# prototypefund/your-voice-TTS

Hardware: AMD Instinct MI355X
Metric: mel-frames/sec + RTF, Tacotron2 + 60-iter Griffin-Lim, LJSpeech (higher is better)
Workload: dtype f32; 1 GPU; configs[1]: Tacotron2 single sentence, HIP decoder loop + HIP Griffin-Lim 60 iters; sentences_per_gpu=1, L=100, gl_iters=60, model_config=config_tacotron2.json + forward_attn_mask (synthesize.py:86), parallelism=single GPU

## Files before the change

your-voice-tts_amd/csrc/resident_decoder.hip:

```cpp
#include "handoff.h"
#include "resident.h"

namespace tts {
namespace {
using namespace handoff;

__device__ __forceinline__ float lstm_cell16(float pre, float& c) {
    const int k = threadIdx.x;
    const float act = (k >> 2) == 2 ? tanh_cell(pre) : sigmoid_cell(pre);
    const float f = dpp_move<0x104, 0xf>(act, 0.f);
    const float g = dpp_move<0x108, 0xf>(act, 0.f);
    const float o = dpp_move<0x10C, 0xf>(act, 0.f);
    const float c2 = f * c + act * g;
    c = c2;
    return o * tanh_cell(c2);
}
__device__ __forceinline__ float sigmoid_fast(float x) {
    return __builtin_amdgcn_rcpf(1.f + __builtin_amdgcn_exp2f(-x * 1.4426950408889634f));
}

__device__ __forceinline__ float dot4(float4 w, float4 x, float acc) {
    acc = fmaf(w.x, x.x, acc);
    acc = fmaf(w.y, x.y, acc);
    acc = fmaf(w.z, x.z, acc);
    return fmaf(w.w, x.w, acc);
}
__device__ __forceinline__ float4 ld4(const float* p) { return *reinterpret_cast<const float4*>(p); }
__device__ __forceinline__ void pin4(float4& a, float4& b, float4& c, float4& d) {
    asm volatile("" : "+v"(a.x), "+v"(a.y), "+v"(a.z), "+v"(a.w), "+v"(b.x), "+v"(b.y), "+v"(b.z), "+v"(b.w), "+v"(c.x),
                 "+v"(c.y), "+v"(c.z), "+v"(c.w), "+v"(d.x), "+v"(d.y), "+v"(d.z), "+v"(d.w));
}
__device__ __forceinline__ float sum32_dpp(float v) {
    v += dpp_move<0x111, 0xf>(v, 0.f);
    v += dpp_move<0x112, 0xf>(v, 0.f);
    v += dpp_move<0x114, 0xf>(v, 0.f);
    v += dpp_move<0x118, 0xf>(v, 0.f);
    v += dpp_move<0x142, 0xa>(v, 0.f);
    return v;
}

__device__ __forceinline__ int res_window(int k, int nn, int L) {
    if (k == 0) return nn >= 2 ? nn - 2 : nn - 2 + L;
    const int clo = nn >= 1 ? nn - 1 : L - 1, chi = min(nn + 2, L - 1);
    const int p = clo + k - 1;
    return p <= chi ? p : -1;
}
__device__ __forceinline__ int res_candidate(int s, int nn, int np, int L) {
    if (s < 5) return res_window(s, nn, L);
    if (s >= 15) return -1;
    const int p = res_window((s - 5) >> 1, np, L);
    if (p < 0) return -1;
    const int q = p + ((s - 5) & 1);
    return q < L ? q : -1;
}

__device__ __forceinline__ int res_part_slot(int sl, int k) { return sl * 32 + k; }

struct ResWin {
    int cx, clo, chi;
    bool in[4];
    bool iscx[4];
    bool pre, post;
};
__device__ __forceinline__ ResWin res_win(int n, int L) {
    ResWin w;
    w.cx = n >= 2 ? n - 2 : n - 2 + L;
    w.clo = n >= 1 ? n - 1 : L - 1;
    w.chi = min(n + 2, L - 1);
#pragma unroll
    for (int k = 0; k < 4; ++k) {
        w.in[k] = w.clo + k <= w.chi;
        w.iscx[k] = w.in[k] && w.clo + k == w.cx;
    }
    w.pre = w.cx < w.clo;
    w.post = w.cx > w.chi;
    return w;
}
__device__ __forceinline__ void res_weights(const ResWin& w, float rm, const float (&c)[4], float& wcx, float (&ww)[4]) {
    float aw[4];
#pragma unroll
    for (int k = 0; k < 4; ++k) aw[k] = (w.in[k] && !w.iscx[k]) ? c[k] : 0.f;
    const float rs = ((aw[0] + aw[1]) + aw[2]) + aw[3];
    const float vx = 0.01f * rm;
    const float denom = rs + vx;
    const float inv = 1.f / denom;
    wcx = vx * inv;
#pragma unroll
    for (int k = 0; k < 4; ++k) ww[k] = aw[k] * inv;
}
__device__ __forceinline__ float res_context(const ResWin& w, float wcx, const float (&ww)[4], float ex,
                                             const float (&erow)[4]) {
    const float px = wcx * ex;
    float ctx = 0.f;
    ctx = w.pre ? ctx + px : ctx;
#pragma unroll
    for (int k = 0; k < 4; ++k) {
        const float s = ctx + (w.iscx[k] ? px : ww[k] * erow[k]);
        ctx = w.in[k] ? s : ctx;
    }
    ctx = w.post ? ctx + px : ctx;
    return ctx;
}
template <bool SEL = false>
__device__ __forceinline__ float res_weight_at(const ResWin& w, float wcx, const float (&ww)[4], int p) {
    int d = p - w.clo;
    if (SEL) asm volatile("" : "+v"(d));
    const float w0 = ww[0], w1 = ww[1], w2 = ww[2], w3 = ww[3];
    float v = w0;
    v = d == 1 ? w1 : v;
    v = d == 2 ? w2 : v;
    v = d >= 3 ? w3 : v;
    v = (d >= 0 && p <= w.chi) ? v : 0.f;
    return p == w.cx ? wcx : v;
}
__device__ __forceinline__ int res_tail_next(const ResWin& w, float wcx, const float (&ww)[4], int L, float& tail) {
    tail = res_weight_at<true>(w, wcx, ww, L - 2) + res_weight_at<true>(w, wcx, ww, L - 1);
    float bv = 0.f;
    int bi = -1;
    auto consider = [&](bool present, int p, float wp) {
        const bool take = present && p <= L - 2 && wp > bv;
        bv = take ? wp : bv;
        bi = take ? p : bi;
    };
    consider(w.pre, w.cx, wcx);
#pragma unroll
    for (int k = 0; k < 4; ++k) consider(w.in[k], w.clo + k, w.iscx[k] ? wcx : ww[k]);
    consider(w.post, w.cx, wcx);
    return bi >= 0 ? bi + 1 : 0;
}

constexpr int SM_WDL = 16 * 16 * 32 * 4;
constexpr int SM_ST = 64;
constexpr int SM_RQ = 4 * 64 * 4;
constexpr int SM_RM = 2 * 6 * 64 * 4 + 2 * 256;
constexpr int SM_PROF = 2 * 16;
constexpr int SM_FLOATS = SM_WDL + HATT + HDEC + (ENC + 16) + PRE + ADIM + 16 + 16 + SM_ST + SM_RQ + SM_RM + SM_PROF + PRE;
static_assert(SM_RQ >= 3 * RES_LMAX + 2 * RES_WAVES + 16 + ADIM, "synthesis form: attention scratch");
static_assert(SM_RQ >= 2 * (RES_LMAX + 32) + RES_LMAX + RES_WAVES, "general attention form: weights, energies");
static_assert(SM_RM >= 2 * 6 * 64 * 4 + RES_LMAX + 32, "general attention form: cumulative weights");
static_assert(HDEC >= 4 * RES_LMAX, "full evaluation: four waves' partials in xh_dec");
static_assert(RES_LMAX == 4 * 64 && RES_LMAX == 32 * RES_WAVES, "4 positions per lane, one per wave of 32 CUs");

template <bool PROF, bool GEN>
__global__ __launch_bounds__(RES_THREADS, 1) void resident_decoder_kernel(const ResArgs a) {
    const int c = blockIdx.x;
    const int tid = threadIdx.x, lane = tid & 63;
    const int wave = __builtin_amdgcn_readfirstlane(tid >> 6);
    const int r = tid >> 5, ks = tid & 31;
    extern __shared__ __align__(16) float sm[];
    float4* wdl = reinterpret_cast<float4*>(sm);
    float* xh_att = sm + SM_WDL;
    float* xh_dec = xh_att + HATT;
    float* xctx = xh_dec + HDEC;
    float* xpre = xctx + ENC + 16;
    float* xq = xpre + PRE;
    float* gates = xq + ADIM;
    int* flags = reinterpret_cast<int*>(gates + 16);
    float* st = gates + 32;
    float* rq = st + SM_ST;
    float* rm = rq + SM_RQ;
    float* abuf = rq;
    float* an = abuf + 2 * RES_LMAX;
    float* scr = an + RES_LMAX;
    float* xv = scr + 2 * RES_WAVES + 16;
    long long* pacc = reinterpret_cast<long long*>(rm + SM_RM);
    float* xp1 = rm + SM_RM + SM_PROF;
    constexpr int GW_PAD = RES_LMAX + 32;
    float* gw = rq;
    float* geg = rq + 2 * GW_PAD;
    float* gts = geg + RES_LMAX;
    float* gcum = rm + 2 * 6 * 64 * 4;
    bool prof = false;
    long long plast = 0;
    long long* trace = PROF && a.prof ? a.prof + 2 * RES_PHASES + (size_t)c * RES_TRACE_STEPS * RES_TRACE_EV : nullptr;
#define RES_EV(t, k)                                                                                \
    if (PROF && trace && (t) < RES_TRACE_STEPS) trace[(t) * RES_TRACE_EV + (k)] = (long long)wall_clock64();
#define RES_MARK(k)                                     \
    if (PROF && prof && tid == 0) {                     \
        const long long now = (long long)wall_clock64(); \
        pacc[k] += now - plast;                         \
        plast = now;                                    \
    }

    float4 wa[14], wdc[4];
    constexpr int KF = HDEC + ENC;
    {
        const float4* p = a.w.wa + (size_t)c * 14 * RES_THREADS + tid;
#pragma unroll
        for (int i = 0; i < 14; ++i) wa[i] = p[(size_t)i * RES_THREADS];
        const float4* q = a.w.wdc + (size_t)c * 4 * RES_THREADS + tid;
#pragma unroll
        for (int i = 0; i < 4; ++i) wdc[i] = q[(size_t)i * RES_THREADS];
        if (wave == 2 && c < a.nmel)
            for (int i = 0; i < 6; ++i) reinterpret_cast<float4*>(rm)[i * 64 + lane] = ld4(a.w.wf + (size_t)c * KF + i * 256 + lane * 4);
        const float4* l = a.w.wdl + (size_t)c * (SM_WDL / 4);
        for (int i = tid; i < SM_WDL / 4; i += RES_THREADS) wdl[i] = l[i];
    }
    if (tid < 16) {
        st[tid] = a.w.ba[c * 16 + tid];
        st[16 + tid] = a.w.bd[c * 16 + tid];
    }
    if (tid < 4) {
        st[32 + tid] = a.c_att[4 * c + tid];
        st[36 + tid] = a.c_dec[4 * c + tid];
    }
    if (tid == 0) st[48] = c < a.nmel ? a.w.bf[c] : 0.f;
    if (tid == 1) st[49] = a.w.bf[a.nmel + PRE];
    for (int k = tid; k < HATT; k += RES_THREADS) {
        xh_att[k] = a.h_att[a.hps + k];
        xh_dec[k] = a.h_dec[a.hps + k];
    }
    for (int k = tid; k < ENC; k += RES_THREADS) xctx[k] = a.xa[PRE + k];
    if (tid == 0) {
        flags[0] = 0;
        flags[1] = 0;
        flags[5] = 0;
        for (int k = 0; k < RES_PHASES; ++k) pacc[k] = 0;
    }
    __syncthreads();
    const long long tmo = a.timeout_ticks;
    int xcc;
    asm volatile("s_getreg_b32 %0, hwreg(HW_REG_XCC_ID)" : "=s"(xcc));
    xcc &= 7;
    const unsigned setup_tag = (a.salt << 14) | 0x3FFFu;
    if (tid == 0) publish(a.gran + GR_SETUP + c, setup_tag, __int_as_float(xcc));
    if (wave == 0) {
        float v4[4];
        const bool ok = sweep<4, !GEN>(a.gran, setup_tag, v4, [&](int i) { return GR_SETUP + lane * 4 + i; }, tmo);
        int rank = 0, nx = 0, nmin = RES_CUS, nmax = 0;
        const int xref = __builtin_amdgcn_readfirstlane(__float_as_int(v4[0]) & 7);
        for (int k = 0; k < 8; ++k) {
            int cnt = 0;
#pragma unroll
            for (int i = 0; i < 4; ++i) {
                const int x = __float_as_int(v4[i]) & 7;
                cnt += __popcll(__ballot(x == k));
                if (k == xcc) rank += __popcll(__ballot(x == k && lane * 4 + i < c));
            }
            if (k == xcc) nx = cnt;
            if (cnt > 0) nmin = min(nmin, cnt);
            nmax = max(nmax, cnt);
        }
        if (GEN && nmax > RES_MIN_CUS_PER_XCD) nmin = 0;
        if (lane == 0) {
            int* fl = reinterpret_cast<int*>(flags);
            fl[2] = rank;
            fl[3] = nx;
            fl[4] = xref;
            if (!ok) { flags[1] = 1; fail(a.status, 6); }
            else if (nmin < RES_MIN_CUS_PER_XCD) { flags[1] = 1; fail(a.status, RES_STATUS_PLACEMENT); }
        }
    }
    __syncthreads();
    if (flags[1]) return;
    const int rank = flags[2], nx = flags[3];
    const int p2lo = rank * PRE / nx, p2hi = (rank + 1) * PRE / nx;
    const int r0 = p2lo + wave;
    const bool has_row = r0 < p2hi;
    const float4 wp0 = has_row ? ld4(a.w.w2 + r0 * PRE + lane * 4) : float4{0.f, 0.f, 0.f, 0.f};
    const float bp1 = has_row ? a.w.bf[a.nmel + r0] : 0.f;
    const float bp2 = has_row ? a.w.b2[r0] : 0.f;
    const float* w1p = a.w.wf + (size_t)(a.nmel + (has_row ? r0 : 0)) * KF + lane * 4;
    const bool stop_cu = rank == 0;
    if (stop_cu && wave == 3)
        for (int i = 0; i < 6; ++i)
            reinterpret_cast<float4*>(rm)[(6 + i) * 64 + lane] = ld4(a.w.wf + (size_t)(a.nmel + PRE) * KF + i * 256 + lane * 4);
    const int qrow = GEN ? 4 * rank + (wave >> 1) : rank + 32 * (wave >> 1), qhalf = wave & 1;
    const float4 wq0 = ld4(a.w.wq + qrow * HATT + qhalf * 512 + lane * 4);
    const float4 wq1 = ld4(a.w.wq + qrow * HATT + qhalf * 512 + 256 + lane * 4);
    const int L = a.L;
    const bool xlog = xcc == flags[4];
    const bool att_log = !GEN && xlog && rank == nx - 1;
    prof = PROF && a.prof != nullptr && a.prof_marks && (c == 0 || att_log);
    if (prof && tid == 0) plast = (long long)wall_clock64();
    int n = 0, n_prev = 0;
    float ufa = 0.f, vb = 0.f, ex = 0.f, erow[4] = {0.f, 0.f, 0.f, 0.f}, ptc = 0.f;
    const auto renc = __builtin_amdgcn_make_buffer_rsrc(const_cast<float*>(a.enc), (short)0, L * ENC * 4, 0x00020000);
    const auto rpt = __builtin_amdgcn_make_buffer_rsrc(const_cast<float*>(a.Pt), (short)0, ADIM * a.Lcap * 4, 0x00020000);
    auto prefetch_rows = [&](int nn) {
        const int cx = nn >= 2 ? nn - 2 : nn - 2 + L, clo = nn >= 1 ? nn - 1 : L - 1, chi = min(nn + 2, L - 1);
        ex = __uint_as_float(__builtin_amdgcn_raw_buffer_load_b32(renc, (cx * ENC + tid) * 4, 0, VOLATILE_AUX));
#pragma unroll
        for (int k = 0; k < 4; ++k)
            erow[k] = __uint_as_float(__builtin_amdgcn_raw_buffer_load_b32(
                renc, clo + k <= chi ? ((clo + k) * ENC + tid) * 4 : OOB_OFF, 0, VOLATILE_AUX));
    };
    auto advance_rows = [&](int from, int nn) {
        if (nn == from) return;
        if (nn == from + 1 && from >= 1) {
            ex = erow[0];
            erow[0] = erow[1];
            erow[1] = erow[2];
            erow[2] = erow[3];
            erow[3] = __uint_as_float(__builtin_amdgcn_raw_buffer_load_b32(
                renc, nn + 2 <= L - 1 ? ((nn + 2) * ENC + tid) * 4 : OOB_OFF, 0, VOLATILE_AUX));
        } else {
            prefetch_rows(nn);
        }
    };
    if constexpr (!GEN) {
        n = a.nidx[0];
        ufa = a.u[0];
        vb = a.v_b[0];
        for (int j = tid; j < L; j += RES_THREADS) abuf[j] = a.alpha[j];
        if (tid < ADIM) xv[tid] = a.v[tid];
        prefetch_rows(n);
    }
    const int gf = GEN ? a.gen : 0;
    const int s_e = GR_EX + xcc * RES_LMAX;
    float gu = 0.5f, gtb = 0.f;
    int gwin = -1, gn = 1;
    float gv0 = 0.f, gv1 = 0.f, gp0 = 0.f, gp1 = 0.f, gl0 = 0.f, gl1 = 0.f;
    float gtw[3];
#pragma unroll
    for (int k = 0; k < 3; ++k) gtw[k] = 0.f;
    auto gen_location = [&](const float* wrow) {
        const int pe = rank + 32 * wave;
        if (pe >= L) return;
        const float* src = (lane < 32 ? wrow : gcum) + pe + 1;
        const float4* wc = reinterpret_cast<const float4*>(a.loc_conv) + lane * 8;
        float sacc = 0.f;
#pragma unroll
        for (int q = 0; q < 8; q += 2) {
            const float4 w0 = wc[q], w1_ = wc[q + 1];
            sacc = fmaf(w0.x, src[4 * q], sacc);
            sacc = fmaf(w0.y, src[4 * q + 1], sacc);
            sacc = fmaf(w0.z, src[4 * q + 2], sacc);
            sacc = fmaf(w0.w, src[4 * q + 3], sacc);
            sacc = fmaf(w1_.x, src[4 * q + 4], sacc);
            sacc = fmaf(w1_.y, src[4 * q + 5], sacc);
            sacc = fmaf(w1_.z, src[4 * q + 6], sacc);
            sacc = fmaf(w1_.w, src[4 * q + 7], sacc);
            asm volatile("" ::: "memory");
        }
        const float tot = sacc + __shfl_xor(sacc, 32, 64);
        const float4* wd0 = reinterpret_cast<const float4*>(a.loc_dense + lane * NLOC);
        const float4* wd1 = reinterpret_cast<const float4*>(a.loc_dense + (lane + 64) * NLOC);
        float l0 = 0.f, l1 = 0.f;
#pragma unroll
        for (int q = 0; q < 8; ++q) {
            const float4 u0 = wd0[q], u1 = wd1[q];
            const float f0 = __int_as_float(__builtin_amdgcn_readlane(__float_as_int(tot), 4 * q));
            const float f1 = __int_as_float(__builtin_amdgcn_readlane(__float_as_int(tot), 4 * q + 1));
            const float f2 = __int_as_float(__builtin_amdgcn_readlane(__float_as_int(tot), 4 * q + 2));
            const float f3 = __int_as_float(__builtin_amdgcn_readlane(__float_as_int(tot), 4 * q + 3));
            l0 = fmaf(u0.x, f0, l0); l0 = fmaf(u0.y, f1, l0); l0 = fmaf(u0.z, f2, l0); l0 = fmaf(u0.w, f3, l0);
            l1 = fmaf(u1.x, f0, l1); l1 = fmaf(u1.y, f1, l1); l1 = fmaf(u1.z, f2, l1); l1 = fmaf(u1.w, f3, l1);
            asm volatile("" ::: "memory");
        }
        gl0 = l0;
        gl1 = l1;
    };
    if constexpr (GEN) {
        vb = a.v_b[0];
        gu = a.u[0];
        gn = a.nidx[0];
        if (gf & GEN_WINDOW) gwin = a.win0[0];
        if (gf & GEN_TA) {
            gtb = a.ta_b[0];
#pragma unroll
            for (int k = 0; k < 3; ++k) gtw[k] = a.ta_w[3 * tid + k];
        }
        gv0 = a.v[lane];
        gv1 = a.v[lane + 64];
        const int pe = rank + 32 * wave;
        if (pe < L) {
            gp0 = a.Pt[(int64_t)lane * a.Lcap + pe];
            gp1 = a.Pt[(int64_t)(lane + 64) * a.Lcap + pe];
        }
        for (int k = tid; k < GW_PAD; k += RES_THREADS) {
            const int j = k - 16;
            const bool ok = j >= 0 && j < L;
            gw[k] = ok ? a.alpha[j] : 0.f;
            gw[GW_PAD + k] = ok && (gf & GEN_LOCATION) ? a.att_w0[j] : 0.f;
            gcum[k] = ok && (gf & GEN_LOCATION) ? a.att_cum0[j] : 0.f;
        }
        __syncthreads();
        if (gf & GEN_LOCATION) gen_location(gw + GW_PAD);
    }
    const bool stop_lane = stop_cu && wave == 3 && lane == 0;
    if (stop_lane) {
        reinterpret_cast<int*>(st)[50] = a.flag1[0];
        reinterpret_cast<int*>(st)[51] = a.count[0];
    }
    u64* Gx = a.gran + GR_PRE2X + xcc * PRE;
    u64* Gq = a.gran + GR_QX + xcc * 2 * ADIM;
    u64* Gc = a.gran + GR_CTXX + xcc * GR_CTXX_STRIDE;
    u64* G1 = a.gran + GR_P1X + xcc * GR_P1X_STRIDE;
    const auto rg = __builtin_amdgcn_make_buffer_rsrc(a.gran, (short)0, 2 * GR_TOTAL * 8, 0x00020000);
    const int s_x = GR_PRE2X + xcc * PRE, s_q = GR_QX + xcc * 2 * ADIM, s_c = GR_CTXX + xcc * GR_CTXX_STRIDE,
              s_1 = GR_P1X + xcc * GR_P1X_STRIDE;
    const int pk = wave * 64 + lane;
    auto mel_row = [&](int tt) {
        if (c >= a.nmel) return;
        const float4* wm = reinterpret_cast<const float4*>(rm) + lane;
        float sm_ = 0.f;
#pragma unroll
        for (int i = 0; i < 4; ++i) sm_ = dot4(wm[i * 64], ld4(xh_dec + i * 256 + lane * 4), sm_);
#pragma unroll
        for (int i = 4; i < 6; ++i) sm_ = dot4(wm[i * 64], ld4(xctx + (i - 4) * 256 + lane * 4), sm_);
        sm_ = wave_sum_dpp(sm_);
        if (lane == 0 && tt < a.hist_cap) a.mel_hist[(int64_t)tt * a.nmel + c] = sm_ + st[48];
    };
#define RES_ATT_PARTIAL(out)                                                                                        \
    {                                                                                                               \
        float aa[2] = {0.f, 0.f};                                                                                   \
        _Pragma("unroll") for (int i = 2; i < 6; ++i)                                                               \
            aa[i & 1] = dot4(wa[i], ld4(xctx + (i - 2) * 128 + ks * 4), aa[i & 1]);                                 \
        _Pragma("unroll") for (int i = 6; i < 10; ++i)                                                              \
            aa[i & 1] = dot4(wa[i], ld4(xh_att + (i - 6) * 128 + ks * 4), aa[i & 1]);                               \
        asm volatile("" ::: "memory");                         \
        _Pragma("unroll") for (int i = 10; i < 14; ++i)                                                             \
            aa[i & 1] = dot4(wa[i], ld4(xh_att + (i - 6) * 128 + ks * 4), aa[i & 1]);                               \
        out = aa[0] + aa[1];                                                                                        \
    }
#define RES_DEC_PARTIAL(out)                                                                                        \
    {                                                                                                               \
        float ad[2] = {0.f, 0.f};                                                                                   \
        _Pragma("unroll 2") for (int i = 8; i < 16; ++i)                                                            \
            ad[i & 1] = dot4(wdl[(i * 16 + r) * 32 + ks], ld4(xh_dec + (i - 8) * 128 + ks * 4), ad[i & 1]);         \
        out = ad[0] + ad[1];                                                                                        \
    }
    float acc_a_next = 0.f;
    if constexpr (!GEN) RES_ATT_PARTIAL(acc_a_next)
    int t = 0;
    for (;; ++t) {
        u64* G = a.gran + (t & 1) * GR_TOTAL;
        u64* const gxs = GEN ? Gx + (t & 1) * GR_TOTAL : G + s_x;
        u64* const gqs = GEN ? Gq + (t & 1) * GR_TOTAL : G + s_q;
        u64* const gcs = GEN ? Gc + (t & 1) * GR_TOTAL : G + s_c;
        u64* const g1s = GEN ? G1 + (t & 1) * GR_TOTAL : G + s_1;
        const unsigned E = (a.salt << 14) | (((unsigned)t & 2047u) << 3);
        const unsigned EP6 = ((a.salt << 14) | (((unsigned)(t - 1) & 2047u) << 3)) + 6u;
        float acc_a, acc_d;
        if constexpr (GEN) {
            RES_ATT_PARTIAL(acc_a)
            RES_DEC_PARTIAL(acc_d)
        } else {
            acc_a = acc_a_next;
        }
        if (tid == 0) { RES_EV(t, 12) }
        if (tid == 192) { RES_EV(t, 13) }
        if (wave < 3) {
            const int gp = s_1 + ((t & 1) ^ 1) * GR_TOTAL;
            bool ok = true;
            if (t == 0) {
                if (wave == 0) {
                    const float4 v = ld4(a.pre1 + lane * 4);
                    xp1[lane * 4] = v.x; xp1[lane * 4 + 1] = v.y; xp1[lane * 4 + 2] = v.z; xp1[lane * 4 + 3] = v.w;
                }
            } else {
                float p0 = 0.f, p1 = 0.f;
                for (int i = 0; i < a.sleep_p1; ++i) __builtin_amdgcn_s_sleep(4);
                if (wave < 2) {
                    ok = sweep_pair(rg, gp + 2 * pk, true, EP6, p0, p1, tmo);
                    xp1[2 * pk] = p0;
                    xp1[2 * pk + 1] = p1;
                } else {
                    ok = sweep_pair(rg, lane == 0 ? gp + PRE : -1, false, EP6, p0, p1, tmo);
                    if (lane == 0 && ok && p0 == 0.f) flags[0] = 1;
                }
            }
            RES_MARK(0);
            if (lane == 0 && !ok) { flags[1] = 1; fail(a.status, 1, t); }
        }
        __syncthreads();
        if (tid == 0) { RES_EV(t, 0) }
        if (flags[0] | flags[1]) break;
        {
            const float4 x = ld4(xp1 + lane * 4);
            u64* gx = gxs;
            if (has_row) {
                const float s0 = wave_sum_dpp(dot4(wp0, x, 0.f));
                if (lane == 0) publish_xcd(gx + r0, E + 1, fmaxf(s0 + bp2, 0.f));
            }
            RES_MARK(1);
            if (wave < 2) {
                for (int i = 0; i < a.sleep_pre2; ++i) __builtin_amdgcn_s_sleep(4);
                float q0, q1;
                const bool ok = sweep_pair(rg, s_x + (t & 1) * GR_TOTAL + 2 * pk, true, E + 1, q0, q1, tmo);
                xpre[2 * pk] = q0;
                xpre[2 * pk + 1] = q1;
                if (!ok && lane == 0) { flags[1] = 1; fail(a.status, 7, t); }
            }
        }
        __syncthreads();
        if (tid == 0) { RES_EV(t, 1) }
        if (flags[1]) break;
        RES_MARK(2);
#pragma unroll
        for (int i = 0; i < 2; ++i) acc_a = dot4(wa[i], ld4(xpre + i * 128 + ks * 4), acc_a);
        acc_a = sum32_dpp(acc_a);
        if (ks == 31) gates[r] = acc_a;
        __syncthreads();
        RES_MARK(3);
        if (tid < 16) {
            float cs = st[32 + (tid & 3)];
            const float h = lstm_cell16(gates[tid] + st[tid], cs);
            if (tid < 4) {
                st[32 + tid] = cs;
                st[40 + tid] = h;
                publish(G + GR_HATT + 4 * c + tid, E + 2, h);
                if (tid == 0) { RES_EV(t, 2) }
            }
        }
        if (!GEN && t > 0) {
            advance_rows(n_prev, n);
            if (wave == 0) {
                const int pos = res_candidate(lane & 15, n, n_prev, L);
                ptc = __uint_as_float(__builtin_amdgcn_raw_buffer_load_b32(
                    rpt, pos >= 0 ? ((rank + 32 * (lane >> 4)) * a.Lcap + pos) * 4 : OOB_OFF, 0, VOLATILE_AUX));
            }
        }
        {
            if constexpr (!GEN) {
                RES_DEC_PARTIAL(acc_d)
                asm volatile("" : "+v"(acc_d));
            }
            if (wave == 4 && t > 0) mel_row(t - 1);
            for (int i = 0; i < a.sleep_hatt; ++i) __builtin_amdgcn_s_sleep(4);
            float h0, h1;
            const bool ok = sweep_pair(rg, (t & 1) * GR_TOTAL + GR_HATT + 2 * pk, true, E + 2, h0, h1, tmo);
            xh_att[2 * pk] = h0;
            xh_att[2 * pk + 1] = h1;
            if (!ok && lane == 0) { flags[1] = 1; fail(a.status, 2, t); }
        }
        __syncthreads();
        if (tid == 0) { RES_EV(t, 3) }
        if (flags[1]) break;
        RES_MARK(4);
        {
            float s = dot4(wq0, ld4(xh_att + qhalf * 512 + lane * 4), 0.f);
            s = dot4(wq1, ld4(xh_att + qhalf * 512 + 256 + lane * 4), s);
            s = wave_sum_dpp(s);
            if constexpr (GEN) {
                if (lane == 0) publish_xcd(gqs + 2 * qrow + qhalf, E + 3, s);
                if (tid == 0) { RES_EV(t, 8) }
            } else {
                if (lane == 0) scr[2 * wave] = s;
            }
        }
        if constexpr (!GEN) {
            __syncthreads();
            if (wave == 0 && t > 0) {
                const int m = lane >> 4;
                const float q = scr[4 * m] + scr[4 * m + 2];
                const float term = __fmul_rn(xv[rank + 32 * m], tanh_fast(__fadd_rn(q, ptc)));
                const float t1 = __shfl(term, (lane & 15) + 16, 64), t2 = __shfl(term, (lane & 15) + 32, 64),
                            t3 = __shfl(term, (lane & 15) + 48, 64);
                const float part = __fadd_rn(__fadd_rn(__fadd_rn(__fadd_rn(0.f, term), t1), t2), t3);
                if (lane < 16) publish_xcd(gcs + res_part_slot(lane, rank), E + 3, part);
                if (tid == 0) { RES_EV(t, 8) }
            }
        }
        if constexpr (!GEN) {
#pragma unroll 1
            for (int h = 0; h < 8; h += 4) {
                float4 wv[4], xx[4];
#pragma unroll
                for (int j = 0; j < 4; ++j) {
                    wv[j] = wdl[((h + j) * 16 + r) * 32 + ks];
                    xx[j] = ld4(xh_att + (h + j) * 128 + ks * 4);
                }
                pin4(wv[0], wv[1], wv[2], wv[3]);
                pin4(xx[0], xx[1], xx[2], xx[3]);
#pragma unroll
                for (int j = 0; j < 4; ++j) acc_d = dot4(wv[j], xx[j], acc_d);
            }
        } else {
#pragma unroll 2
            for (int i = 0; i < 8; ++i) acc_d = dot4(wdl[(i * 16 + r) * 32 + ks], ld4(xh_att + i * 128 + ks * 4), acc_d);
        }
        RES_MARK(5);
        float wcx = 0.f, ww[4] = {0.f, 0.f, 0.f, 0.f};
        if constexpr (GEN) {
            float2 gen_e[4];
#pragma unroll
            for (int i = 0; i < 4; ++i) {
                const int ps = (i >> 1) * 128 + 2 * lane + (i & 1);
                gen_e[i] = __builtin_bit_cast(float2, __builtin_amdgcn_raw_buffer_load_b64(
                    renc, ps < L ? (ps * ENC + 16 * rank + 2 * wave) * 4 : OOB_OFF, 0, VOLATILE_AUX));
            }
            if (wave < 2) {
                for (int i = 0; i < a.sleep_q; ++i) __builtin_amdgcn_s_sleep(1);
                float q0, q1;
                const bool ok = sweep_pair(rg, s_q + (t & 1) * GR_TOTAL + 2 * pk, true, E + 3, q0, q1, tmo);
                xq[pk] = q0 + q1;
                if (!ok && lane == 0) { flags[1] = 1; fail(a.status, 3, t); }
            }
            __syncthreads();
            if (flags[1]) break;
            if (rank + 32 * wave < L) {
                float x0 = xq[lane], x1 = xq[lane + 64];
                if (gf & GEN_LOCATION) {
                    x0 += gl0;
                    x1 += gl1;
                }
                const float e = wave_sum_dpp(gv0 * tanh_fast(x0 + gp0) + gv1 * tanh_fast(x1 + gp1));
                if (lane == 0) publish_xcd(a.gran + (t & 1) * GR_TOTAL + s_e + rank + 32 * wave, E + 7, e + vb);
            }
            if (wave < 2) {
                for (int i = 0; i < a.sleep_e; ++i) __builtin_amdgcn_s_sleep(1);
                const int p0 = 2 * pk;
                float e0 = 0.f, e1 = 0.f;
                const bool ok =
                    sweep_pair(rg, p0 < L ? s_e + (t & 1) * GR_TOTAL + p0 : -1, p0 + 1 < L, E + 7, e0, e1, tmo);
                geg[p0] = e0;
                geg[p0 + 1] = e1;
                if (!ok && lane == 0) { flags[1] = 1; fail(a.status, 8, t); }
            }
            __syncthreads();
            if (flags[1]) break;
            RES_MARK(6);
            const float* wold = gw + (t & 1) * GW_PAD + 16;
            float* wnew = gw + ((t & 1) ^ 1) * GW_PAD + 16;
            int ps[4];
            bool in[4];
            float e[4];
            {
                const float2 g0 = *reinterpret_cast<const float2*>(geg + 2 * lane);
                const float2 g1 = *reinterpret_cast<const float2*>(geg + 128 + 2 * lane);
                e[0] = g0.x; e[1] = g0.y; e[2] = g1.x; e[3] = g1.y;
            }
#pragma unroll
            for (int i = 0; i < 4; ++i) {
                ps[i] = (i >> 1) * 128 + 2 * lane + (i & 1);
                in[i] = ps[i] < L;
                if (!in[i]) e[i] = -INFINITY;
            }
            if (gf & GEN_WINDOW) {
                const int back = gwin - 2, front = gwin + 6;
#pragma unroll
                for (int i = 0; i < 4; ++i)
                    if (in[i] && ((back > 0 && ps[i] < back) || (front < L && ps[i] >= front))) e[i] = -INFINITY;
                if (gwin == -1) {
                    const float m = wave_max_dpp(fmaxf(fmaxf(e[0], e[1]), fmaxf(e[2], e[3])));
                    if (lane == 0) e[0] = m;
                }
                float bv = e[0];
                int bi = ps[0];
#pragma unroll
                for (int i = 1; i < 4; ++i)
                    if (e[i] > bv) { bv = e[i]; bi = ps[i]; }
                wave_argmax(bv, bi);
                gwin = __builtin_amdgcn_readfirstlane(bi);
            }
            float al[4];
            if (gf & GEN_SOFTMAX) {
                const float m = wave_max_dpp(fmaxf(fmaxf(e[0], e[1]), fmaxf(e[2], e[3])));
#pragma unroll
                for (int i = 0; i < 4; ++i) al[i] = in[i] ? expf(e[i] - m) : 0.f;
            } else {
#pragma unroll
                for (int i = 0; i < 4; ++i) al[i] = in[i] ? sigmoidf_(e[i]) : 0.f;
            }
            {
                const float S = wave_sum_dpp((al[0] + al[1]) + (al[2] + al[3]));
#pragma unroll
                for (int i = 0; i < 4; ++i) al[i] = al[i] / S;
            }
            if ((gf & GEN_LOCATION) && wave == 0) {
                float2* c01 = reinterpret_cast<float2*>(gcum + 16 + 2 * lane);
                float2* c23 = reinterpret_cast<float2*>(gcum + 16 + 128 + 2 * lane);
                const float2 o01 = *c01, o23 = *c23;
                *c01 = float2{o01.x + al[0], o01.y + al[1]};
                *c23 = float2{o23.x + al[2], o23.y + al[3]};
            }
            float w[4];
            if (gf & GEN_FORWARD) {
                float an[4];
#pragma unroll
                for (int i = 0; i < 4; ++i) {
                    const float ao = wold[ps[i]], pv = wold[ps[i] - 1];
                    const float mix = __fadd_rn(__fadd_rn(__fmul_rn(1.f - gu, ao), __fmul_rn(gu, pv)), 1e-8f);
                    an[i] = in[i] ? __fmul_rn(mix, al[i]) : 0.f;
                }
                if (gf & GEN_MASK) {
                    const float rmax = wave_max_dpp(fmaxf(fmaxf(in[0] ? an[0] : -INFINITY, in[1] ? an[1] : -INFINITY),
                                                          fmaxf(in[2] ? an[2] : -INFINITY, in[3] ? an[3] : -INFINITY)));
                    const int cx = gn >= 2 ? gn - 2 : gn - 2 + L, lo = gn >= 1 ? gn - 1 : L - 1;
#pragma unroll
                    for (int i = 0; i < 4; ++i) {
                        const bool keep = in[i] && ps[i] < gn + 3 && ps[i] >= lo;
                        an[i] = ps[i] == cx ? 0.01f * rmax : (keep ? an[i] : 0.f);
                    }
                }
                const float denom = wave_sum_dpp((an[0] + an[1]) + (an[2] + an[3]));
#pragma unroll
                for (int i = 0; i < 4; ++i) w[i] = in[i] ? an[i] / denom : 0.f;
                if (gf & GEN_MASK) {
                    float bv = -1.f;
                    int bi = 0x7fffffff;
#pragma unroll
                    for (int i = 0; i < 4; ++i)
                        if (ps[i] <= L - 2 && w[i] > bv) { bv = w[i]; bi = ps[i]; }
                    wave_argmax(bv, bi);
                    gn = __builtin_amdgcn_readfirstlane(bv > 0.f ? bi + 1 : 0);
                }
            } else {
#pragma unroll
                for (int i = 0; i < 4; ++i) w[i] = al[i];
            }
            RES_MARK(7);
            const float tail = wave_sum_dpp(((ps[0] >= L - 2 && in[0] ? w[0] : 0.f) + (ps[1] >= L - 2 && in[1] ? w[1] : 0.f)) +
                                            ((ps[2] >= L - 2 && in[2] ? w[2] : 0.f) + (ps[3] >= L - 2 && in[3] ? w[3] : 0.f)));
            float c0 = 0.f, c1 = 0.f;
#pragma unroll
            for (int i = 0; i < 4; ++i) {
                c0 = fmaf(w[i], gen_e[i].x, c0);
                c1 = fmaf(w[i], gen_e[i].y, c1);
            }
            c0 = wave_sum_dpp(c0);
            c1 = wave_sum_dpp(c1);
            {
                u64* gcx = gcs;
                if (lane < 2) publish_xcd(gcx + 16 * rank + 2 * wave + lane, E + 4, lane ? c1 : c0);
                if (rank == 0 && wave == 0 && lane == 2) publish_xcd(gcx + ENC, E + 4, tail);
            }
            if (tid == 0) { RES_EV(t, 11) }
            RES_MARK(8);
            if (wave == 0) {
                *reinterpret_cast<float2*>(wnew + 2 * lane) = float2{w[0], w[1]};
                *reinterpret_cast<float2*>(wnew + 128 + 2 * lane) = float2{w[2], w[3]};
                if (xlog && rank == 0 && t < a.hist_cap) {
#pragma unroll
                    for (int i = 0; i < 4; ++i)
                        if (ps[i] < a.Lalign) a.align_hist[(int64_t)t * a.Lalign + ps[i]] = w[i];
                }
            }
        }
        if constexpr (!GEN) {
            const float* aold = abuf + (t & 1) * RES_LMAX;
            float* candv = scr + 2 * RES_WAVES;
            const ResWin win = res_win(n, L);
            const int sl = tid >> 5, sub = tid & 31;
            const int pos = t > 0 ? res_candidate(sl, n, n_prev, L) : -1;
            const float a_pos = pos >= 0 ? aold[pos] : 0.f, a_prev = pos > 0 ? aold[pos - 1] : 0.f;
            const float mix = __fadd_rn(__fadd_rn(__fmul_rn(1.f - ufa, a_pos), __fmul_rn(ufa, a_prev)), 1e-8f);
            RES_MARK(9);
            bool full = t == 0;
            float rm = -INFINITY;
            float cw[4] = {0.f, 0.f, 0.f, 0.f};
            if (!full) {
                for (int i = 0; i < a.sleep_q; ++i) __builtin_amdgcn_s_sleep(1);
                float part = 0.f;
                const bool ok = sweep_one(rg, s_c + (t & 1) * GR_TOTAL + res_part_slot(sl, sub), E + 3, part, tmo);
                if (!ok && lane == 0) { flags[1] = 1; fail(a.status, 10, t); }
                if (tid == 0) { RES_EV(t, 9) }
                RES_MARK(6);
                const float e = sum32_dpp(part);
                if (sub == 31) {
                    const float v = pos >= 0 ? __fmul_rn(mix, sigmoid_fast(e + vb)) : -INFINITY;
                    if (pos >= 0) an[pos] = v;
                    candv[sl] = v;
                }
                __syncthreads();
                if (tid == 0) { RES_EV(t, 10) }
                if (flags[1]) break;
                RES_MARK(14);
                const float cand = candv[lane & 15];
                rm = wave_max_dpp(cand);
                full = !(rm >= 1e-8f);
#pragma unroll
                for (int k = 0; k < 4; ++k) cw[k] = __int_as_float(__builtin_amdgcn_readlane(__float_as_int(cand), 1 + k));
            }
            if (full) {
                const unsigned F = (a.salt << 14) | (((unsigned)flags[5] & 2047u) << 3) | 3u;
                if (lane == 0) publish_xcd(gqs + 2 * qrow + qhalf, F, scr[2 * wave]);
                if (wave < 2) {
                    float q0, q1;
                    const bool ok = sweep_pair(rg, s_q + (t & 1) * GR_TOTAL + 2 * pk, true, F, q0, q1, tmo);
                    xq[pk] = q0 + q1;
                    if (!ok && lane == 0) { flags[1] = 1; fail(a.status, 3, t); }
                }
                __syncthreads();
                if (flags[1]) break;
                if (tid == 0) flags[5] += 1;
                float xqd[16];
#pragma unroll
                for (int dd = 0; dd < 16; ++dd) xqd[dd] = xq[16 * wave + dd];
                float* red = xh_dec;
                const int j = tid;
                float e = 0.f;
#pragma unroll 1
                for (int h = 0; h < 2; ++h) {
                    if ((wave >> 2) == h) {
#pragma unroll 1
                        for (int jj = lane; jj < L; jj += 64) {
                            float s = 0.f;
#pragma unroll
                            for (int dd = 0; dd < 16; ++dd) {
                                const int d = 16 * wave + dd;
                                s += xv[d] * tanh_fast(xqd[dd] + a.Pt[(int64_t)d * a.Lcap + jj]);
                            }
                            red[(wave & 3) * RES_LMAX + jj] = s;
                        }
                    }
                    __syncthreads();
                    if (j < L) {
#pragma unroll
                        for (int w = 0; w < 4; ++w) e += red[w * RES_LMAX + j];
                    }
                    __syncthreads();
                }
                float anj = -INFINITY;
                if (j < L) {
                    const float sg = sigmoid_fast(e + vb);
                    const float prev = j > 0 ? aold[j - 1] : 0.f;
                    const float mixj = __fadd_rn(__fadd_rn(__fmul_rn(1.f - ufa, aold[j]), __fmul_rn(ufa, prev)), 1e-8f);
                    anj = __fmul_rn(mixj, sg);
                    an[j] = anj;
                }
                const float wmax = wave_max_dpp(anj);
                if (lane == 0) scr[2 * wave + 1] = wmax;
                __syncthreads();
                rm = -INFINITY;
#pragma unroll
                for (int k = 0; k < RES_WAVES; ++k) rm = fmaxf(rm, scr[2 * k + 1]);
#pragma unroll
                for (int k = 0; k < 4; ++k) cw[k] = an[win.clo + k];
            }
            RES_MARK(7);
            res_weights(win, rm, cw, wcx, ww);
            const float ctx = res_context(win, wcx, ww, ex, erow);
            RES_MARK(15);
            xctx[tid] = ctx;
        }
        float4 w1[6];
        if constexpr (GEN) {
#pragma unroll
            for (int i = 0; i < 6; ++i) w1[i] = ld4(w1p + i * 256);
        }
        if constexpr (GEN) {
            if (wave < 5) {
                const int gc = s_c + (t & 1) * GR_TOTAL;
                for (int i = 0; i < a.sleep_ctx; ++i) __builtin_amdgcn_s_sleep(4);
                float c0 = 0.f, c1 = 0.f;
                const bool ok = wave < 4 ? sweep_pair(rg, gc + 2 * pk, true, E + 4, c0, c1, tmo)
                                         : sweep_pair(rg, lane == 0 ? gc + ENC : -1, false, E + 4, c0, c1, tmo);
                if (wave < 4) {
                    xctx[2 * pk] = c0;
                    xctx[2 * pk + 1] = c1;
                } else if (lane == 0) {
                    xctx[ENC] = c0;
                }
                if (!ok && lane == 0) { flags[1] = 1; fail(a.status, 4, t); }
            }
        }
        __syncthreads();
        if (tid == 0) { RES_EV(t, 4) }
        if (flags[1]) break;
        if constexpr (GEN) { RES_MARK(10); }
#pragma unroll
        for (int i = 0; i < 4; ++i) acc_d = dot4(wdc[i], ld4(xctx + i * 128 + ks * 4), acc_d);
        acc_d = sum32_dpp(acc_d);
        if (ks == 31) gates[r] = acc_d;
        __syncthreads();
        RES_MARK(11);
        if constexpr (!GEN) {
#pragma unroll
            for (int i = 0; i < 6; ++i) w1[i] = ld4(w1p + i * 256);
        }
        if (tid < 16) {
            float cs = st[36 + (tid & 3)];
            const float h = lstm_cell16(gates[tid] + st[16 + tid], cs);
            if (tid < 4) {
                st[36 + tid] = cs;
                st[44 + tid] = h;
                publish(G + GR_HDEC + 4 * c + tid, E + 5, h);
                if (tid == 0) { RES_EV(t, 5) }
            }
        }
        if constexpr (GEN) {
            if (gf & GEN_TA) {
                float pta = 0.f;
#pragma unroll
                for (int k = 0; k < 3; ++k) {
                    const int idx = 3 * tid + k;
                    pta = fmaf(gtw[k], idx < ENC ? xctx[idx] : xh_att[idx - ENC], pta);
                }
                pta = wave_sum_dpp(pta);
                if (lane == 0) gts[wave] = pta;
            }
            if (gf & GEN_LOCATION) gen_location(gw + ((t & 1) ^ 1) * GW_PAD);
        }
        if constexpr (!GEN) {
            const ResWin win = res_win(n, L);
            if (wave == RES_WAVES - 1) {
                float tail;
                const int n_next = res_tail_next(win, wcx, ww, L, tail);
                if (lane == 0) {
                    xctx[ENC] = tail;
                    flags[6] = n_next;
                }
            }
            float* anew = abuf + ((t & 1) ^ 1) * RES_LMAX;
            const float wdef = tid < L ? res_weight_at(win, wcx, ww, tid) : 0.f;
            if (tid < L) anew[tid] = wdef;
            if (att_log && t < a.hist_cap && tid < a.Lalign) a.align_hist[(int64_t)t * a.Lalign + tid] = wdef;
        }
        {
            if constexpr (!GEN) {
                RES_ATT_PARTIAL(acc_a_next)
                asm volatile("" : "+v"(acc_a_next));
            }
            for (int i = 0; i < a.sleep_hdec; ++i) __builtin_amdgcn_s_sleep(4);
            float h0, h1;
            const bool ok = sweep_pair(rg, (t & 1) * GR_TOTAL + GR_HDEC + 2 * pk, true, E + 5, h0, h1, tmo);
            xh_dec[2 * pk] = h0;
            xh_dec[2 * pk + 1] = h1;
            if (!ok && lane == 0) { flags[1] = 1; fail(a.status, 5, t); }
        }
        __syncthreads();
        if (tid == 0) { RES_EV(t, 6) }
        if (flags[1]) break;
        if constexpr (!GEN) {
            n_prev = n;
            n = flags[6];
        }
        if constexpr (GEN) {
            if (gf & GEN_TA) {
                float sta = gts[0];
#pragma unroll
                for (int k = 1; k < RES_WAVES; ++k) sta += gts[k];
                gu = sigmoidf_(sta + gtb);
            }
        }
        RES_MARK(12);
        long long m0 = 0;
        if (prof && tid == 128) m0 = (long long)wall_clock64();
        {
            const bool stw = stop_cu && wave == 3;
            const float4* wsr = reinterpret_cast<const float4*>(rm) + 6 * 64 + lane;
            float s = 0.f, ss = 0.f;
#pragma unroll
            for (int i = 0; i < 4; ++i) {
                const float4 x = ld4(xh_dec + i * 256 + lane * 4);
                s = dot4(w1[i], x, s);
                if (stw) ss = dot4(wsr[i * 64], x, ss);
            }
#pragma unroll
            for (int i = 4; i < 6; ++i) {
                const float4 x = ld4(xctx + (i - 4) * 256 + lane * 4);
                s = dot4(w1[i], x, s);
                if (stw) ss = dot4(wsr[i * 64], x, ss);
            }
            s = wave_sum_dpp(s);
            u64* g1 = g1s;
            if (has_row && lane == 0) {
                const float p = fmaxf(s + bp1, 0.f);
                publish_xcd(g1 + r0, E + 6, p);
                if (wave == 0) { RES_EV(t, 7) }
                if (xlog) a.pre1[r0] = p;
            }
            if (stw) {
                ss = wave_sum_dpp(ss);
                if (lane == 0) {
                    const float stv = sigmoidf_(ss + st[49]);
                    if (xlog && t < a.hist_cap) a.stop_hist[t] = stv;
                    const float tail = xctx[ENC];
                    int* sst = reinterpret_cast<int*>(st);
                    const int f1 = sst[50] | ((tail > 0.8f && t > L) ? 1 : 0);
                    sst[50] = f1;
                    int nd = 0;
                    if (f1 && t > 2 * L) {
                        sst[51] += 1;
                        if (sst[51] > 20) nd = 1;
                    } else if (t + 1 == a.max_steps) {
                        nd = 1;
                    }
                    if (!nd && t + 1 >= a.hist_cap) {
                        nd = 1;
                        fail(a.status, 100);
                    }
                    if (nd && xlog) {
                        a.done[0] = 1;
                        a.n_steps[0] = t + 1;
                    }
                    publish_xcd(g1 + PRE, E + 6, nd ? 0.f : 1.f);
                }
            }
        }
        if (prof && tid == 128) pacc[13] += (long long)wall_clock64() - m0;
    }
    if (flags[1]) return;
    if (wave == 4 && t > 0) mel_row(t - 1);
    if (prof && tid == 0)
        for (int k = 0; k < RES_PHASES; ++k) a.prof[(c == 0 ? 0 : 1) * RES_PHASES + k] = pacc[k];
    const int pl = (t - 1) & 1;
    if (tid < 4) {
        a.h_att[pl * a.hps + 4 * c + tid] = st[40 + tid];
        a.c_att[4 * c + tid] = st[32 + tid];
        a.h_dec[pl * a.hps + 4 * c + tid] = st[44 + tid];
        a.c_dec[4 * c + tid] = st[36 + tid];
    }
    if (c == 0)
        for (int k = tid; k < ENC; k += RES_THREADS) a.xa[(1 - pl) * a.xps + PRE + k] = xctx[k];
}

__global__ void res_pack_wa(const float* wih, const float* whh, float4* out) {
    const int64_t idx = (int64_t)blockIdx.x * blockDim.x + threadIdx.x;
    if (idx >= (int64_t)RES_CUS * 14 * RES_THREADS) return;
    const int tid = idx % RES_THREADS, i4 = (idx / RES_THREADS) % 14, c = idx / (14 * RES_THREADS);
    const int r = tid >> 5, ks = tid & 31, row = (r >> 2) * HATT + 4 * c + (r & 3);
    float v[4];
    for (int j = 0; j < 4; ++j) {
        const int k = i4 * 128 + ks * 4 + j;
        v[j] = k < XA ? wih[(int64_t)row * XA + k] : whh[(int64_t)row * HATT + (k - XA)];
    }
    out[idx] = float4{v[0], v[1], v[2], v[3]};
}
__global__ void res_pack_wd(const float* wih, const float* whh, float4* wdl, float4* wdc) {
    const int64_t idx = (int64_t)blockIdx.x * blockDim.x + threadIdx.x;
    constexpr int PER = 16 * 16 * 32 + 4 * RES_THREADS;
    if (idx >= (int64_t)RES_CUS * PER) return;
    const int c = idx / PER, e = idx % PER;
    float v[4];
    if (e < 16 * 16 * 32) {
        const int i4 = e / 512, r = (e / 32) % 16, ks = e % 32;
        const int row = (r >> 2) * HDEC + 4 * c + (r & 3);
        for (int j = 0; j < 4; ++j) {
            const int k = i4 * 128 + ks * 4 + j;
            v[j] = k < HATT ? wih[(int64_t)row * (HATT + ENC) + k] : whh[(int64_t)row * HDEC + (k - HATT)];
        }
        wdl[(int64_t)c * 8192 + e] = float4{v[0], v[1], v[2], v[3]};
    } else {
        const int f = e - 16 * 16 * 32, i4 = f / RES_THREADS, tid = f % RES_THREADS;
        const int r = tid >> 5, ks = tid & 31, row = (r >> 2) * HDEC + 4 * c + (r & 3);
        for (int j = 0; j < 4; ++j) v[j] = wih[(int64_t)row * (HATT + ENC) + HATT + i4 * 128 + ks * 4 + j];
        wdc[((int64_t)c * 4 + i4) * RES_THREADS + tid] = float4{v[0], v[1], v[2], v[3]};
    }
}
__global__ void res_pack_bias(const float* abih, const float* abhh, const float* dbih, const float* dbhh, float* ba,
                              float* bd) {
    const int idx = blockIdx.x * blockDim.x + threadIdx.x;
    if (idx < RES_CUS * 16) {
        const int c = idx / 16, r = idx % 16, row = (r >> 2) * HATT + 4 * c + (r & 3);
        ba[idx] = abih[row] + abhh[row];
        bd[idx] = dbih[row] + dbhh[row];
    }
}

__global__ void res_pack_loc(const float* w, float* out) {
    const int idx = blockIdx.x * blockDim.x + threadIdx.x;
    if (idx >= 2 * NLOC * 32) return;
    const int k = idx & 31, f = (idx >> 5) % NLOC, c = idx / (32 * NLOC);
    out[idx] = k < KLOC ? w[(f * 2 + c) * KLOC + k] : 0.f;
}

}

hipError_t resident_pack_location(const float* w, float* out, hipStream_t s) {
    hipLaunchKernelGGL(res_pack_loc, dim3((2 * NLOC * 32 + 255) / 256), dim3(256), 0, s, w, out);
    return hipGetLastError();
}

void resident_weight_floats(size_t* wa, size_t* wdl, size_t* wdc) {
    *wa = (size_t)RES_CUS * 14 * RES_THREADS * 4;
    *wdl = (size_t)RES_CUS * 16 * 16 * 32 * 4;
    *wdc = (size_t)RES_CUS * 4 * RES_THREADS * 4;
}

hipError_t resident_pack(const ResSrc& s, const ResWeights& w, hipStream_t st) {
    auto blocks = [](int64_t n) { return dim3((unsigned)((n + 255) / 256)); };
    hipLaunchKernelGGL(res_pack_wa, blocks((int64_t)RES_CUS * 14 * RES_THREADS), dim3(256), 0, st, s.a_wih, s.a_whh,
                       w.wa);
    hipLaunchKernelGGL(res_pack_wd, blocks((int64_t)RES_CUS * (8192 + 4 * RES_THREADS)), dim3(256), 0, st, s.d_wih,
                       s.d_whh, w.wdl, w.wdc);
    (void)hipMemcpyAsync(w.w2, s.w_pre2, sizeof(float) * PRE * PRE, hipMemcpyDeviceToDevice, st);
    if (s.b_pre2)
        (void)hipMemcpyAsync(w.b2, s.b_pre2, sizeof(float) * PRE, hipMemcpyDeviceToDevice, st);
    else
        (void)hipMemsetAsync(w.b2, 0, sizeof(float) * PRE, st);
    (void)hipMemcpyAsync(w.wq, s.w_q, sizeof(float) * ADIM * HATT, hipMemcpyDeviceToDevice, st);
    (void)hipMemcpyAsync(w.wf, s.wf, sizeof(float) * s.nrows * (HDEC + ENC), hipMemcpyDeviceToDevice, st);
    (void)hipMemcpyAsync(w.bf, s.bf, sizeof(float) * s.nrows, hipMemcpyDeviceToDevice, st);
    hipLaunchKernelGGL(res_pack_bias, blocks(RES_CUS * 16), dim3(256), 0, st, s.a_bih, s.a_bhh, s.d_bih, s.d_bhh, w.ba,
                       w.bd);
    return hipGetLastError();
}

size_t resident_smem_bytes() { return (size_t)SM_FLOATS * sizeof(float); }

hipError_t resident_prepare() {
    const void* fns[] = {reinterpret_cast<const void*>(&resident_decoder_kernel<false, false>),
                         reinterpret_cast<const void*>(&resident_decoder_kernel<true, false>),
                         reinterpret_cast<const void*>(&resident_decoder_kernel<false, true>),
                         reinterpret_cast<const void*>(&resident_decoder_kernel<true, true>)};
    for (const void* fn : fns) {
        hipError_t e = hipFuncSetAttribute(fn, hipFuncAttributeMaxDynamicSharedMemorySize, (int)resident_smem_bytes());
        if (e != hipSuccess) return e;
    }
    return hipSuccess;
}

hipError_t launch_resident(const ResArgs& a, hipStream_t s, bool* launched) {
    *launched = false;
    if (a.L < 2 || a.L > RES_LMAX || a.nmel > RES_CUS || a.nmel + PRE + 1 != a.nrows) return hipErrorInvalidValue;
    ResArgs arg = a;
    void* args[] = {&arg};
    if (a.gen && ((a.gen & GEN_TA) && !(a.ta_w && a.ta_b))) return hipErrorInvalidValue;
    if (a.gen && ((a.gen & GEN_LOCATION) && !(a.att_w0 && a.att_cum0 && a.loc_conv && a.loc_dense)))
        return hipErrorInvalidValue;
    if (a.gen && (a.gen & GEN_WINDOW) && !a.win0) return hipErrorInvalidValue;
    const void* fn = a.gen ? (a.prof ? reinterpret_cast<const void*>(&resident_decoder_kernel<true, true>)
                                     : reinterpret_cast<const void*>(&resident_decoder_kernel<false, true>))
                           : (a.prof ? reinterpret_cast<const void*>(&resident_decoder_kernel<true, false>)
                                     : reinterpret_cast<const void*>(&resident_decoder_kernel<false, false>));
    return launch_persistent(fn, dim3(RES_CUS), dim3(RES_THREADS), args, resident_smem_bytes(), s, launched);
}

}
```

Measured before the change: 102,000 mel-frames/s.

## Issue next-step encoder-row and attention-P loads from non-polling waves at step end

Moves the encoder-row advance load and the Pt candidate load out of the critical path after the attention LSTM. They are now issued at the end of the previous step by waves that do not poll, and handed to the polling waves and wave 0 through a new LDS slot before the existing barrier. This is meant to hide global-load latency on the waves that run the cross-CU sweeps. It costs extra LDS and registers and ties correctness to the wave-role split.

```diff
diff --git a/your-voice-tts_amd/csrc/resident_decoder.hip b/your-voice-tts_amd/csrc/resident_decoder.hip
--- a/your-voice-tts_amd/csrc/resident_decoder.hip
+++ b/your-voice-tts_amd/csrc/resident_decoder.hip
@@ -134,8 +134,12 @@
 constexpr int SM_RQ = 4 * 64 * 4;
 constexpr int SM_RM = 2 * 6 * 64 * 4 + 2 * 256;
 constexpr int SM_PROF = 2 * 16;
-constexpr int SM_FLOATS = SM_WDL + HATT + HDEC + (ENC + 16) + PRE + ADIM + 16 + 16 + SM_ST + SM_RQ + SM_RM + SM_PROF + PRE;
-static_assert(SM_RQ >= 3 * RES_LMAX + 2 * RES_WAVES + 16 + ADIM, "synthesis form: attention scratch");
+constexpr int RES_POLL_WAVES = 3;
+constexpr int SM_OPR = RES_POLL_WAVES * 64;
+constexpr int SM_FLOATS = SM_WDL + HATT + HDEC + (ENC + 16) + PRE + ADIM + 16 + 16 + SM_ST + SM_RQ + SM_RM + SM_PROF + PRE + SM_OPR;
+static_assert(SM_FLOATS * 4 <= 160 * 1024, "the CU's LDS");
+static_assert(SM_RQ >= 3 * RES_LMAX + 2 * RES_WAVES + 16 + ADIM + 64, "synthesis form: attention scratch, P slot");
+static_assert(2 * RES_POLL_WAVES <= RES_WAVES - 1, "a loading wave per polling wave, one for P");
 static_assert(SM_RQ >= 2 * (RES_LMAX + 32) + RES_LMAX + RES_WAVES, "general attention form: weights, energies");
 static_assert(SM_RM >= 2 * 6 * 64 * 4 + RES_LMAX + 32, "general attention form: cumulative weights");
 static_assert(HDEC >= 4 * RES_LMAX, "full evaluation: four waves' partials in xh_dec");
@@ -163,8 +167,10 @@
     float* an = abuf + 2 * RES_LMAX;
     float* scr = an + RES_LMAX;
     float* xv = scr + 2 * RES_WAVES + 16;
+    float* xpt = xv + ADIM;
     long long* pacc = reinterpret_cast<long long*>(rm + SM_RM);
     float* xp1 = rm + SM_RM + SM_PROF;
+    float* xrow = xp1 + PRE;
     constexpr int GW_PAD = RES_LMAX + 32;
     float* gw = rq;
     float* geg = rq + 2 * GW_PAD;
@@ -275,6 +281,7 @@
     if (prof && tid == 0) plast = (long long)wall_clock64();
     int n = 0, n_prev = 0;
     float ufa = 0.f, vb = 0.f, ex = 0.f, erow[4] = {0.f, 0.f, 0.f, 0.f}, ptc = 0.f;
+    float op_own = 0.f, op_row = 0.f, op_pt = 0.f;
     const auto renc = __builtin_amdgcn_make_buffer_rsrc(const_cast<float*>(a.enc), (short)0, L * ENC * 4, 0x00020000);
     const auto rpt = __builtin_amdgcn_make_buffer_rsrc(const_cast<float*>(a.Pt), (short)0, ADIM * a.Lcap * 4, 0x00020000);
     auto prefetch_rows = [&](int nn) {
@@ -284,19 +291,6 @@
         for (int k = 0; k < 4; ++k)
             erow[k] = __uint_as_float(__builtin_amdgcn_raw_buffer_load_b32(
                 renc, clo + k <= chi ? ((clo + k) * ENC + tid) * 4 : OOB_OFF, 0, VOLATILE_AUX));
-    };
-    auto advance_rows = [&](int from, int nn) {
-        if (nn == from) return;
-        if (nn == from + 1 && from >= 1) {
-            ex = erow[0];
-            erow[0] = erow[1];
-            erow[1] = erow[2];
-            erow[2] = erow[3];
-            erow[3] = __uint_as_float(__builtin_amdgcn_raw_buffer_load_b32(
-                renc, nn + 2 <= L - 1 ? ((nn + 2) * ENC + tid) * 4 : OOB_OFF, 0, VOLATILE_AUX));
-        } else {
-            prefetch_rows(nn);
-        }
     };
     if constexpr (!GEN) {
         n = a.nidx[0];
@@ -492,6 +486,12 @@
         for (int i = 0; i < 2; ++i) acc_a = dot4(wa[i], ld4(xpre + i * 128 + ks * 4), acc_a);
         acc_a = sum32_dpp(acc_a);
         if (ks == 31) gates[r] = acc_a;
+        if constexpr (!GEN) {
+            if (t > 0) {
+                if (wave >= RES_POLL_WAVES && wave < 2 * RES_POLL_WAVES) xrow[tid - 64 * RES_POLL_WAVES] = op_row;
+                if (wave == 2 * RES_POLL_WAVES) xpt[lane] = op_pt;
+            }
+        }
         __syncthreads();
         RES_MARK(3);
         if (tid < 16) {
@@ -504,12 +504,19 @@
                 if (tid == 0) { RES_EV(t, 2) }
             }
         }
-        if (!GEN && t > 0) {
-            advance_rows(n_prev, n);
-            if (wave == 0) {
-                const int pos = res_candidate(lane & 15, n, n_prev, L);
-                ptc = __uint_as_float(__builtin_amdgcn_raw_buffer_load_b32(
-                    rpt, pos >= 0 ? ((rank + 32 * (lane >> 4)) * a.Lcap + pos) * 4 : OOB_OFF, 0, VOLATILE_AUX));
+        if constexpr (!GEN) {
+            if (t > 0) {
+                if (n == n_prev + 1 && n_prev >= 1) {
+                    ex = erow[0];
+                    erow[0] = erow[1];
+                    erow[1] = erow[2];
+                    erow[2] = erow[3];
+                    if (wave < RES_POLL_WAVES) erow[3] = xrow[tid];
+                    else erow[3] = op_own;
+                } else if (n != n_prev) {
+                    prefetch_rows(n);
+                }
+                if (wave == 0) ptc = xpt[lane];
             }
         }
         {
@@ -982,6 +989,23 @@
             }
         }
         if (prof && tid == 128) pacc[13] += (long long)wall_clock64() - m0;
+        if constexpr (!GEN) {
+            if (wave >= RES_POLL_WAVES) {
+                if (n == n_prev + 1 && n_prev >= 1) {
+                    const int ro = n + 2 <= L - 1 ? ((n + 2) * ENC + tid) * 4 : OOB_OFF;
+                    op_own = __uint_as_float(__builtin_amdgcn_raw_buffer_load_b32(renc, ro, 0, VOLATILE_AUX));
+                    if (wave < 2 * RES_POLL_WAVES)
+                        op_row = __uint_as_float(__builtin_amdgcn_raw_buffer_load_b32(
+                            renc, n + 2 <= L - 1 ? ro - 256 * RES_POLL_WAVES : OOB_OFF, 0, VOLATILE_AUX));
+                }
+                if (wave == 2 * RES_POLL_WAVES) {
+                    const int pos = res_candidate(lane & 15, n, n_prev, L);
+                    op_pt = __uint_as_float(__builtin_amdgcn_raw_buffer_load_b32(
+                        rpt, pos >= 0 ? ((rank + 32 * (lane >> 4)) * a.Lcap + pos) * 4 : OOB_OFF, 0, VOLATILE_AUX));
+                    if (lane == 0) { RES_EV(t, 14) }
+                }
+            }
+        }
     }
     if (flags[1]) return;
     if (wave == 4 && t > 0) mel_row(t - 1);
```

Result: faster. 103,400 mel-frames/s, median of 6 (+1.3%).
